# yxyxcyx/Real-Time-Recommendation-System-with-Feature-Store

Measured on AMD Instinct MI355X. Metric: user-item pairs scored/sec (train) + top-K queries/sec, emb_dim=128, higher is better.
Workload: dtype f32; 1 GPU; C2: MovieLens-1M two-tower train step, emb 128, batch 1024, 16 negatives, hidden [256,128], dropout 0.2, tau 0.05, Adam+clip; global_batch=1024, emb_dim=128, num_negatives=16, parallelism=dp1

## Files before the change

### include/rtrec_hip.h

```cpp
#ifndef RTREC_HIP_H
#define RTREC_HIP_H

#include <stddef.h>
#include <stdint.h>

#ifdef __cplusplus
extern "C" {
#endif

typedef enum {
    RT_OK = 0,
    RT_ERR_INVALID = -1,
    RT_ERR_UNSUPPORTED = -2,
    RT_ERR_WORKSPACE = -3,
    RT_ERR_HIP = -4
} rt_status;

typedef enum { RT_F32 = 0, RT_F16 = 1, RT_BF16 = 2 } rt_dtype;

typedef enum {
    RT_ACT_RELU = 0,
    RT_ACT_GELU = 1,
    RT_ACT_LEAKY_RELU = 2,
    RT_ACT_TANH = 3,
// ... 157 lines not shown
    const float* bn_gamma;
    float* dgamma;
    float* dbeta;
    const float* src; int64_t src_rows; int ld_src; const int64_t* ids;
    int prev_mode; int prev_act;
    const float* prev_mean; const float* prev_invstd;
    const float* prev_gamma; const float* prev_beta;
    float prev_drop_p; uint64_t prev_drop_seed; const uint64_t* seed_offset;
    float* g_prev;
    double* g_prev_stats;
    float* dsrc;
    int64_t seg_split;
    double* dbias_slots;
    const float* wt;
    int fuse_dz;
    const float* a_in;
    float* dw_part;
    const float* fold_src;
    float* fold_dst;
    int64_t fold_words;
    int fold_splits;
    int fold_in;
    const uint16_t* wt_planes;
} rt_linear_bwd_args;

int rt_linear_bwd_f32(const rt_linear_bwd_args* args, void* stream);
int rt_linear_bwd_dz_fused(const rt_linear_bwd_args* args, int n_args);
int rt_linear_bwd_dw_splits(const rt_linear_bwd_args* args, int n_args, int64_t* splits);
int rt_linear_bwd_dz_f32(const rt_linear_bwd_args* args, void* stream);
int rt_linear_bwd_dw_f32(const rt_linear_bwd_args* args, void* stream);
int rt_linear_fwd_f32_multi(const rt_linear_fwd_args* args, int n_args, void* stream);
int rt_linear_bwd_dz_f32_multi(const rt_linear_bwd_args* args, int n_args, void* stream);
int rt_linear_bwd_dw_f32_multi(const rt_linear_bwd_args* args, int n_args, void* stream);
int rt_linear_bwd_dw_f32_joint(const rt_linear_bwd_args* args, int n_args, void* stream);
int rt_linear_bwd_dw_joint_splits(const rt_linear_bwd_args* args, int n_args, int64_t* splits);

size_t rt_twotower_loss_workspace_bytes(int64_t b, int d);
int rt_twotower_loss_fwd_bwd(const void* u, const void* p, const void* q, int dtype, int64_t b,
                             int d, int n_neg, float inv_tau, const float* user_bias,
                             const float* item_bias, float w_explicit, float w_in_batch,
                             double* loss_out, float* du, float* dp, float* dq, float* d_user_bias,
                             float* d_item_bias, void* workspace, size_t workspace_bytes, void* stream);

int rt_twotower_loss_fwd(const void* u, const void* p, const void* q, int dtype, int64_t b, int d,
                         int n_neg, float inv_tau, const float* user_bias, const float* item_bias,
                         float w_explicit, float w_in_batch, double* loss_out, void* workspace,
                         size_t workspace_bytes, void* stream);

size_t rt_inbatch_loss_workspace_bytes(int64_t b, int64_t n_items, int d);
int rt_inbatch_loss_fwd_bwd(const void* u, const void* p, int dtype, int64_t b, int64_t n_items, int d,
                            int64_t label_offset, float inv_tau, double* loss_out, float* du, float* dp,
                            void* workspace, size_t workspace_bytes, void* stream);

int rt_similarity_f32(const float* u, const float* v, int64_t b, int d, float inv_tau,
                      const float* user_bias, const float* item_bias, float* out, void* stream);

#define RT_GRAD_FOLD_MAX 8
typedef struct {
    const float* part;
    int64_t dst_off;
    int64_t words;
    int splits;
    int tensor;
} rt_grad_fold;
int rt_grad_sqnorm(const float* grads, const int64_t* offsets, int n_tensors, double* sumsq_out,
// ... 54 lines not shown
```

### real-time-recommendation-system-with-feature-store_amd/csrc/loss.hip

```cpp
#include <float.h>

#include "rt_common.h"
#include "split3.h"

namespace rt {
size_t ib16_workspace_bytes(int64_t b, int64_t nx, int d);
int ib16_run(const void* u, const void* p, int dtype, int64_t b, int64_t nx, int d, int64_t off, float inv_tau,
             double* loss_out, float* du, float* dp, void* ws, size_t ws_bytes, hipStream_t st);
namespace loss {

typedef float f32x16 __attribute__((ext_vector_type(16)));
constexpr int RB = 32;
constexpr int kMaxD = 256;
constexpr int kMaxNeg = 64;
constexpr int NG = 16;


__device__ __forceinline__ int tile_row(int r, int h) { return (r & 3) + 8 * (r >> 2) + 4 * h; }

struct Args {
    const void* u; const void* p; const void* q;
    int64_t b; int d; int n_neg; float inv_tau;
    const float* ub; const float* ib;
    float we, wb;
    double* loss;
    float* du; float* dp; float* dq; float* dub; float* dib;
    float2* part;
    float* diag;
    float* expl;
    float* dposv;
    int64_t nx;
    int64_t off;
    int n_split;
    int ib_blocks;
    bool grad;
};

constexpr int SPAN = 256;
constexpr int LDP = 4;

template <typename T>
__device__ __forceinline__ float4 load4(const T* __restrict__ p) {
    if constexpr (sizeof(T) == 4) {
        return *reinterpret_cast<const float4*>(p);
    } else {
        const uint2 r = *reinterpret_cast<const uint2*>(p);
        const T* e = reinterpret_cast<const T*>(&r);
        return make_float4(to_f32(e[0]), to_f32(e[1]), to_f32(e[2]), to_f32(e[3]));
    }
}

template <int DP, typename T>
__device__ __forceinline__ void load_rows(const T* __restrict__ M, int64_t r0, int64_t n, int D,
                                          float4 (&v)[DP / 8]) {
    const int lane = threadIdx.x & 63;
#pragma unroll
    for (int u = 0; u < DP / 8; ++u) {
        const int e = lane + 64 * u;
// ... 171 lines not shown
            }
        }
    }
    wave_lds_sync();
    float se = expf(pos - mx);
    for (int j = 0; j < a.n_neg; ++j) se += expf(negs[w][j] - mx);
    const float lse = mx + logf(se);
    const float dpos = a.we * inv_b * (expf(pos - lse) - 1.f);
    if (lane == 0) {
        a.expl[i] = lse - pos;
        a.dposv[i] = dpos;
    }
    if (!a.grad) return;
    float duv[V];
#pragma unroll
    for (int t = 0; t < V; ++t) duv[t] = dpos * pv[t];
    for (int g0 = 0; g0 < a.n_neg; g0 += NG) {
        if (a.n_neg > NG) load_q(g0);
#pragma unroll
        for (int jj = 0; jj < NG; ++jj) {
            const int j = g0 + jj;
            if (j >= a.n_neg) break;
            const float dn = a.we * inv_b * expf(negs[w][j] - lse);
            float* dqr = a.dq + (i * a.n_neg + j) * D;
#pragma unroll
            for (int t = 0; t < V; ++t) {
                const int dd = lane + 64 * t;
                if (dd < D) {
                    duv[t] += dn * qv[jj][t];
                    dqr[dd] = dn * uv[t] * a.inv_tau;
                }
            }
        }
    }
#pragma unroll
    for (int t = 0; t < V; ++t) {
        const int dd = lane + 64 * t;
        if (dd < D) {
            a.du[i * D + dd] = duv[t] * a.inv_tau;
            a.dp[i * D + dd] = dpos * uv[t] * a.inv_tau;
        }
    }
}

__device__ __forceinline__ float combine_lse(const float2* part, int n_split, int64_t b, int64_t i) {
    float mm = -INFINITY;
    for (int s = 0; s < n_split; ++s) mm = fmaxf(mm, part[static_cast<int64_t>(s) * b + i].x);
    float ll = 0.f;
    for (int s = 0; s < n_split; ++s) {
        const float2 v = part[static_cast<int64_t>(s) * b + i];
        if (v.x != -INFINITY) ll += v.y * expf(v.x - mm);
    }
    return mm + logf(ll);
// ... 163 lines not shown
    hipLaunchKernelGGL((loss::loss_bwd_kernel<DP, T>), grid2, dim3(256), lds, st, a, wb_eff, true);
    return check_launch("loss_bwd_kernel");
}

template <typename T>
int launch_loss_d(const loss::Args& a, int dp32, dim3 grid1, dim3 grid2, float wb_eff, hipStream_t st) {
    switch (dp32) {
        case 32: return launch_loss<32, T>(a, grid1, grid2, wb_eff, st);
        case 64: return launch_loss<64, T>(a, grid1, grid2, wb_eff, st);
        case 96:
        case 128: return launch_loss<128, T>(a, grid1, grid2, wb_eff, st);
        default: return launch_loss<256, T>(a, grid1, grid2, wb_eff, st);
    }
}

size_t loss_ws_bytes(int64_t b, int64_t nx) {
    const int64_t n_split = (nx + loss::SPAN - 1) / loss::SPAN;
    return static_cast<size_t>(n_split) * b * sizeof(float2) + 3 * static_cast<size_t>(b) * sizeof(float);
}

int run_loss(const void* u, const void* p, const void* q, int dtype, int64_t b, int64_t nx, int64_t off, int d,
             int n_neg, float inv_tau, const float* ub, const float* ib, float we, float wb, double* loss_out,
             float* du, float* dp, float* dq, float* dub, float* dib, void* ws, size_t ws_bytes, void* stream,
             bool grad) {
    if (dtype != RT_F32 && dtype != RT_F16 && dtype != RT_BF16) return RT_ERR_INVALID;
    if (b <= 0 || d <= 0 || n_neg < 0 || !u || !p || !loss_out) return RT_ERR_INVALID;
    if (nx < b || off < 0 || off + b > nx) return RT_ERR_INVALID;
    if (d % 8 != 0 || d > loss::kMaxD || n_neg > loss::kMaxNeg) return RT_ERR_UNSUPPORTED;
    if (n_neg > 0 && !q) return RT_ERR_INVALID;
    if (grad && (!du || !dp || (n_neg > 0 && !dq))) return RT_ERR_INVALID;
    const int n_split = static_cast<int>((nx + loss::SPAN - 1) / loss::SPAN);
    if (!ws || ws_bytes < loss_ws_bytes(b, nx)) return RT_ERR_WORKSPACE;
    if ((reinterpret_cast<uintptr_t>(u) | reinterpret_cast<uintptr_t>(p)) & 15) return RT_ERR_INVALID;
    float2* part = reinterpret_cast<float2*>(ws);
    float* diag = reinterpret_cast<float*>(part + static_cast<size_t>(n_split) * b);
    const float wb_eff = n_neg > 0 ? wb : 1.f;
    const float we_eff = n_neg > 0 ? we : 0.f;
    const bool want_ib = wb_eff != 0.f;
    loss::Args a{u, p, q, b, d, n_neg, inv_tau, ub, ib, we_eff, wb_eff, loss_out, du, dp, dq, dub, dib, part, diag,
                 diag + b, diag + 2 * b, nx, off, n_split, want_ib ? n_split : 0, grad};
    hipStream_t st = as_stream(stream);
    if (grad && nx != b) {
        if (hipMemsetAsync(dp, 0, static_cast<size_t>(nx) * d * sizeof(float), st) != hipSuccess)
            return check_launch("hipMemsetAsync(dp)");
    }
    const int64_t big = nx > b ? nx : b;
    const int dp32 = (d + 31) / 32 * 32;
    const unsigned y2 = static_cast<unsigned>((big + loss::SPAN - 1) / loss::SPAN);
    const dim3 grid1(static_cast<unsigned>((b + loss::RB - 1) / loss::RB), a.ib_blocks + 8);
    const dim3 grid2(static_cast<unsigned>((big + loss::RB - 1) / loss::RB), want_ib ? y2 : 1,
                     (grad && want_ib) ? 2 : 1);
    switch (dtype) {
        case RT_F32: return launch_loss_d<float>(a, dp32, grid1, grid2, wb_eff, st);
        case RT_F16: return launch_loss_d<__half>(a, dp32, grid1, grid2, wb_eff, st);
        default: return launch_loss_d<__hip_bfloat16>(a, dp32, grid1, grid2, wb_eff, st);
    }
}
}

extern "C" size_t rt_twotower_loss_workspace_bytes(int64_t b, int d) {
    (void)d;
    if (b <= 0) return 256;
    return loss_ws_bytes(b, b) + 256;
// ... 11 lines not shown
    if (dtype == RT_F16 || dtype == RT_BF16) {
        if (b <= 0 || d <= 0 || !u || !p || !loss_out) return RT_ERR_INVALID;
        if (n_items < b || label_offset < 0 || label_offset + b > n_items) return RT_ERR_INVALID;
        if (d % 8 != 0 || d > loss::kMaxD) return RT_ERR_UNSUPPORTED;
        if ((du == nullptr) != (dp == nullptr)) return RT_ERR_INVALID;
        if ((reinterpret_cast<uintptr_t>(u) | reinterpret_cast<uintptr_t>(p)) & 15) return RT_ERR_INVALID;
        return ib16_run(u, p, dtype, b, n_items, d, label_offset, inv_tau, loss_out, du, dp, workspace,
                        workspace_bytes, as_stream(stream));
    }
    return run_loss(u, p, nullptr, dtype, b, n_items, label_offset, d, 0, inv_tau, nullptr, nullptr, 0.f, 1.f,
                    loss_out, du, dp, nullptr, nullptr, nullptr, workspace, workspace_bytes, stream, du != nullptr);
}


extern "C" int rt_twotower_loss_fwd_bwd(const void* u, const void* p, const void* q, int dtype, int64_t b, int d,
                                        int n_neg, float inv_tau, const float* user_bias, const float* item_bias,
                                        float w_explicit, float w_in_batch, double* loss_out, float* du, float* dp,
                                        float* dq, float* d_user_bias, float* d_item_bias, void* workspace,
                                        size_t workspace_bytes, void* stream) {
    return run_loss(u, p, q, dtype, b, b, 0, d, n_neg, inv_tau, user_bias, item_bias, w_explicit, w_in_batch,
                    loss_out, du, dp, dq, d_user_bias, d_item_bias, workspace, workspace_bytes, stream, true);
}

extern "C" int rt_twotower_loss_fwd(const void* u, const void* p, const void* q, int dtype, int64_t b, int d,
                                    int n_neg, float inv_tau, const float* user_bias, const float* item_bias,
                                    float w_explicit, float w_in_batch, double* loss_out, void* workspace,
                                    size_t workspace_bytes, void* stream) {
    return run_loss(u, p, q, dtype, b, b, 0, d, n_neg, inv_tau, user_bias, item_bias, w_explicit, w_in_batch,
                    loss_out, nullptr, nullptr, nullptr, nullptr, nullptr, workspace, workspace_bytes, stream, false);
}

extern "C" int rt_similarity_f32(const float* u, const float* v, int64_t b, int d, float inv_tau,
                                 const float* user_bias, const float* item_bias, float* out, void* stream) {
    if (b < 0 || d <= 0 || !u || !v || !out) return RT_ERR_INVALID;
    if ((user_bias == nullptr) != (item_bias == nullptr)) return RT_ERR_INVALID;
    if (b == 0) return RT_OK;
    hipLaunchKernelGGL(loss::similarity_kernel, dim3(static_cast<unsigned>((b + 3) / 4)), dim3(256), 0,
                       as_stream(stream), u, v, b, d, inv_tau, user_bias, item_bias, out);
    return check_launch("similarity_kernel");
}
```

### real-time-recommendation-system-with-feature-store_amd/csrc/mlp.hip

```cpp
#include "rt_common.h"
#include "split3.h"

namespace rt {
namespace mlp {

typedef float f32x16 __attribute__((ext_vector_type(16)));



constexpr float kNormEps = 1e-12f;

struct FwdLaunch {
    rt_linear_fwd_args a0, a1;
    unsigned split;
};
struct BwdLaunch {
    rt_linear_bwd_args a0, a1;
    unsigned split;
    int64_t rps0, rps1;
    unsigned tn0, tk0, tn1, tk1;
    bool vec0, vec1;
    int ngroups;
    unsigned ksplit = 1;
};
// ... 179 lines not shown
                s2 += v2[sl];
            }
            const double md = s1 / static_cast<double>(ms);
            double vd = s2 / static_cast<double>(ms) - md * md;
            vd = vd > 0.0 ? vd : 0.0;
            const float mean = static_cast<float>(md);
            const float invstd = static_cast<float>(1.0 / sqrt(vd + static_cast<double>(a.fin_eps)));
            const float var_f = static_cast<float>(ms > 1 ? vd * static_cast<double>(ms) / static_cast<double>(ms - 1) : vd);
            a.fin_save_mean[sg * n + c] = mean;
            if (a.fin_save_invstd) a.fin_save_invstd[sg * n + c] = invstd;
            if (a.fin_running_mean) {
                const float mo = a.fin_momentum;
                a.fin_running_mean[c] = (1.f - mo) * a.fin_running_mean[c] + mo * mean;
                a.fin_running_var[c] = (1.f - mo) * a.fin_running_var[c] + mo * var_f;
            }
        }
    }
    if (tid == 0 && a.fin_num_batches_tracked) *a.fin_num_batches_tracked += nseg;
}

constexpr int FM = 32;

__host__ __device__ __forceinline__ int pad8(int k) { return (k + 31) / 32 * 32; }

template <int TPW, bool KVEC, bool WPL>
__global__ __launch_bounds__(256) __attribute__((amdgpu_waves_per_eu(TPW == 1 ? 3 : 2))) void linear_fwd_kernel(FwdLaunch L) {
    static_assert(!WPL || (TPW == 1 && KVEC), "split-weight planes: one-tile waves, k % 4 == 0");
    const bool g1 = blockIdx.x >= L.split;
    const rt_linear_fwd_args& a = g1 ? L.a1 : L.a0;
    const unsigned bid = blockIdx.x - (g1 ? L.split : 0u);
    constexpr int NT = 4 * TPW;
    extern __shared__ __attribute__((aligned(16))) float sm[];
    const int k = a.k, n = a.n;
    const int kp = pad8(k), aplane = FM * kp, aw = 3 * aplane / 2;
    const int nch = kp / 8, am = ((nch & -nch) < 16 ? (nch & -nch) : 16) - 1;
    float* scale = sm;
    float* shift = scale + kp;
    float* As = shift + kp;
    uint16_t* const Ap = reinterpret_cast<uint16_t*>(As);
    float* rowpart = As + aw;
    int64_t* srow = reinterpret_cast<int64_t*>(rowpart + NT * FM);

    const int tid = threadIdx.x, lane = tid & 63, w = tid >> 6, h = lane >> 5, c32 = lane & 31;
    const int64_t row0 = static_cast<int64_t>(bid) * FM;
    const int64_t m = a.m;
    auto put_a = [&](int r, int c, float4 o) {
// ... 503 lines not shown
    uint4 pv[TPWK][3], pn[TPWK][3];
    const uint16_t* __restrict__ WtP = a.wt_planes;
    const int64_t tplane = static_cast<int64_t>(k) * n;
    auto load_p = [&](int s, uint4 (&dst)[TPWK][3]) {
#pragma unroll
        for (int i = 0; i < TPWK; ++i) {
            const int kk = (tb + w + 4 * i) * 32 + c32;
            const int nn = s + 8 * h;
            const bool ok = (tb + w + 4 * i) * 32 < k && kk < k && nn < n;
            const uint16_t* q = WtP + (ok ? static_cast<int64_t>(kk) * n + nn : 0);
#pragma unroll
            for (int p = 0; p < 3; ++p)
                dst[i][p] = ok ? *reinterpret_cast<const uint4*>(q + p * tplane) : make_uint4(0u, 0u, 0u, 0u);
        }
    };
    if constexpr (TPWK == 1) {
        if (a.g_prev || a.dsrc) {
            if constexpr (WPL) load_p(0, pn);
            else load_w(0, wn);
        }
    }

    const int l4 = n / 4;
    if (a.grad_mode == 0 && (n % 4) == 0 && l4 <= 64 && (l4 & (l4 - 1)) == 0 && np == n) {
        const int rpp = 64 / l4, sub = lane / l4, li = lane % l4, c = 4 * li;
        float4 lv[8], dv[8];
        float nr[8];
#pragma unroll
        for (int p = 0; p < 8; ++p) {
            const int r = w * 8 + p * rpp + sub;
            const int64_t gr = row0 + r;
            lv[p] = make_float4(0.f, 0.f, 0.f, 0.f);
            dv[p] = lv[p];
            nr[p] = 1.f;
            if (p * rpp < 8 && gr < m) {
                lv[p] = *reinterpret_cast<const float4*>(a.l2_out + gr * n + c);
                dv[p] = *reinterpret_cast<const float4*>(a.dout + gr * n + c);
                nr[p] = a.norms[gr];
            }
        }
#pragma unroll
        for (int p = 0; p < 8; ++p) {
            if (p * rpp >= 8) break;
            const int r = w * 8 + p * rpp + sub;
            const int64_t gr = row0 + r;
            float dot = lv[p].x * dv[p].x + lv[p].y * dv[p].y + lv[p].z * dv[p].z + lv[p].w * dv[p].w;
            for (int o = 1; o < l4; o <<= 1) dot += __shfl_xor(dot, o, 64);
            const bool big = nr[p] > kNormEps;
            const float inv = 1.f / (big ? nr[p] : kNormEps);
            float4 d = make_float4(0.f, 0.f, 0.f, 0.f);
            if (gr < m) {
                d.x = big ? (dv[p].x - lv[p].x * dot) * inv : dv[p].x * inv;
                d.y = big ? (dv[p].y - lv[p].y * dot) * inv : dv[p].y * inv;
                d.z = big ? (dv[p].z - lv[p].z * dot) * inv : dv[p].z * inv;
                d.w = big ? (dv[p].w - lv[p].w * dot) * inv : dv[p].w * inv;
                if (prim) st_act4(a.dz_ws + gr * n + c, d);
            }
            *reinterpret_cast<float4*>(Dz + r * ldz + c) = d;
        }
    } else if (a.grad_mode == 0) {
        for (int rr = w * 8; rr < w * 8 + 8; ++rr) {
            const int64_t gr = row0 + rr;
            if (gr < m) {
                float dot = 0.f;
                for (int c = lane; c < n; c += 64) dot += a.l2_out[gr * n + c] * a.dout[gr * n + c];
                dot = wave_sum(dot);
                const float nrm = a.norms[gr];
                const bool big = nrm > kNormEps;
// ... 795 lines not shown
}

static bool dz_fusable(const rt_linear_bwd_args& a) {
#ifdef RT_NO_DZ_FUSE
    return false;
#endif
    return a.fuse_dz && !a.g_prev && !a.dsrc && a.grad_mode >= 1 && a.grad_mode <= 3 &&
           act_is_piecewise_linear(a.act) && (a.n % 4) == 0 && a.g && a.z &&
           (reinterpret_cast<uintptr_t>(a.g) & 15) == 0 && (reinterpret_cast<uintptr_t>(a.z) & 15) == 0;
}
static bool all_dz_fusable(const rt_linear_bwd_args* args, int n_args) {
    for (int g = 0; g < n_args; ++g)
        if (!dz_fusable(args[g])) return false;
    return true;
}

static int validate_bwd(const rt_linear_bwd_args* args) {
    if (!args) return RT_ERR_INVALID;
    const rt_linear_bwd_args& a = *args;
    if (a.m < 0 || a.k <= 0 || a.n <= 0 || !a.w || !a.dw || !a.dz_ws || !a.src || a.ld_src < a.k)
        return RT_ERR_INVALID;
    const bool need_da = a.g_prev || a.dsrc;
    if (a.n > 2048 || (need_da && a.k > 512)) return RT_ERR_UNSUPPORTED;
    if (a.grad_mode == 0 && (!a.dout || !a.l2_out || !a.norms)) return RT_ERR_INVALID;
    if (a.grad_mode >= 1 && a.grad_mode <= 3 && (!a.g || !a.z)) return RT_ERR_INVALID;
    if ((a.grad_mode == 1 || a.grad_mode == 2) && (!a.g_stats || !a.save_mean || !a.save_invstd || !a.bn_gamma))
        return RT_ERR_INVALID;
    if (a.grad_mode < 0 || a.grad_mode > 3) return RT_ERR_INVALID;
    if (a.seg_split < 0 || (a.seg_split > 0 && (a.seg_split >= a.m || a.seg_split % mlp::FM != 0)))
        return RT_ERR_INVALID;
    if ((a.prev_mode == 1 || a.prev_mode == 2) &&
        (!a.prev_mean || !a.prev_invstd || !a.prev_gamma || !a.prev_beta))
        return RT_ERR_INVALID;
    if (a.fold_src && (!a.fold_dst || a.fold_words % 4 != 0 || a.fold_splits <= 0 || a.fold_in < 0 || a.fold_in > 1 ||
                       (reinterpret_cast<uintptr_t>(a.fold_src) & 15) || (reinterpret_cast<uintptr_t>(a.fold_dst) & 15)))
        return RT_ERR_INVALID;
    if (a.wt_planes && ((a.n % 8) != 0 || (reinterpret_cast<uintptr_t>(a.wt_planes) & 15))) return RT_ERR_INVALID;
    return RT_OK;
}

extern "C" int rt_linear_bwd_dz_f32_multi(const rt_linear_bwd_args* args, int n_args, void* stream) {
    if (!args || n_args < 1 || n_args > 2) return RT_ERR_INVALID;
    int tpwk = 1;
    size_t lds = 0;
    unsigned blocks[2] = {0u, 0u};
    bool wpl = true;
    for (int g = 0; g < n_args; ++g) {
// ... 388 lines not shown
```

### real-time-recommendation-system-with-feature-store_amd/rtrec_amd/models/fused.py

```python
from __future__ import annotations

import ctypes
import itertools
import os
from dataclasses import dataclass, field
from typing import List, Optional

import torch
import torch.nn as nn

from .. import native
from ..native import LinearBwdArgs, LinearFwdArgs, call, ptr
from ..profiling import TIMER

ACT_CODE = {nn.ReLU: 0, nn.GELU: 1, nn.LeakyReLU: 2, nn.Tanh: 3, nn.Sigmoid: 4}
ACT_NONE = 5

_seed_counter = itertools.count(1)


def act_code(mod: Optional[nn.Module]) -> int:
    if mod is None:
        return ACT_NONE
    for cls, code in ACT_CODE.items():
# ... 343 lines not shown
                ctx.norms = norms
            else:
                a.z_out = out.data_ptr()
            ctx.out = out
        layers.append(a)
    return ctx, layers


def chain_backward(blocks: List[Block], ctx: ChainCtx, dout: torch.Tensor, slab: ParamSlab,
                   want_dsrc: bool = False, seed_offset: Optional[torch.Tensor] = None,
                   stats_arena: Optional[torch.Tensor] = None, attach: bool = True) -> Optional[torch.Tensor]:
    layers, dsrc, keep = _backward_plan(blocks, ctx, dout, slab, want_dsrc, seed_offset, stats_arena, attach)
    st = _stream(dout)
    groups = [[a] for a in layers]
    if dw_joint_enabled():
        _launch_bwd_joint(groups, st, None)
        return dsrc
    keep += _plan_partials(groups, dout.device)
    for g in groups:
        _launch_bwd(g, st)
    return dsrc


def chain_backward_pair(first: tuple, second: tuple, fold_sink: Optional["FoldSink"] = None) -> None:
    l1, _, keep1 = _backward_plan(*first)
    l2, _, keep2 = _backward_plan(*second)
    st = _stream(first[2])
    if len(l1) == len(l2):
        groups = [[a, b] for a, b in zip(l1, l2)]
        if dw_joint_enabled():
            _launch_bwd_joint(groups, st, fold_sink)
            return
        keep1 += _plan_partials(groups, first[2].device)
    else:
        groups = [[a] for a in l1 + l2]
    for g in groups:
        _launch_bwd(g, st)


def dw_joint_enabled() -> bool:
    lib = native.lib()
    return (os.environ.get("RTREC_DW_LEGACY", "0") != "1" and hasattr(lib, "rt_linear_bwd_dw_f32_joint")
            and hasattr(lib, "rt_linear_bwd_dw_joint_splits") and hasattr(lib, "rt_linear_bwd_dz_fused"))


class FoldSink:

    def __init__(self, slab: ParamSlab):
        self.slab = slab
        self.buf: Optional[torch.Tensor] = None
        self.retired: list = []
        self.folds: list = []

    def begin(self) -> None:
        self.folds = []

# ... 80 lines not shown
    fused = hasattr(lib, "rt_linear_bwd_dz_fused") and lib.rt_linear_bwd_dz_fused(arr, len(group))
    if not fused:
        _launch_dz(group, st)
    _launch_dw(group, st)


def _launch_dz(group: list, st) -> None:
    da = [a.g_prev is not None or a.dsrc is not None for a in group]
    flops = sum((2.0 if d else 0.0) * a.m * a.k * a.n for a, d in zip(group, da))
    nbytes = sum(4.0 * (3 * a.m * a.n + (2 * a.m * a.k if d else 0) + a.n * a.k) for a, d in zip(group, da))
    with TIMER.region("linear_bwd_dz", flops=flops, bytes_=nbytes):
        call("rt_linear_bwd_dz_f32_multi", (LinearBwdArgs * len(group))(*group), len(group), st)


def _launch_dw(group: list, st) -> None:
    with TIMER.region("linear_bwd_dw", flops=sum(2.0 * a.m * a.k * a.n for a in group),
                      bytes_=sum(4.0 * (a.m * a.n + a.m * a.k + a.n * a.k) for a in group)):
        call("rt_linear_bwd_dw_f32_multi", (LinearBwdArgs * len(group))(*group), len(group), st)


def _backward_plan(blocks: List[Block], ctx: ChainCtx, dout: torch.Tensor, slab: ParamSlab,
                   want_dsrc: bool = False, seed_offset: Optional[torch.Tensor] = None,
                   stats_arena: Optional[torch.Tensor] = None, attach: bool = True):
    dev = dout.device
    dout = dout.contiguous()
    m = ctx.m
    L = len(blocks) - 1
    if attach:
        slab.attach_grads()
    dz_bufs = [torch.empty((m, b.linear.out_features), dtype=torch.float32, device=dev) for b in blocks]
    layers = []
    widths = [b.linear.out_features for b in blocks[:-1]]
    n_seg = 2 if ctx.seg_split else 1
    gst_arena = stats_arena if stats_arena is not None else \
        torch.zeros(stats_arena_size(blocks, n_seg), dtype=torch.float64, device=dev)
    gstats, off = [], 0
    for wdt in widths:
        gstats.append(gst_arena[off:off + n_seg * STAT_SLOTS * 2 * wdt])
        off += n_seg * STAT_SLOTS * 2 * wdt
    bslots = []
    for b in blocks:
        bslots.append(gst_arena[off:off + DBIAS_ROWS * b.linear.out_features])
        off += DBIAS_ROWS * b.linear.out_features
    gs: List[Optional[torch.Tensor]] = [None] * L
    dsrc = torch.empty((m, blocks[0].linear.in_features), dtype=torch.float32, device=dev) if want_dsrc else None
    keep = [dout, gst_arena] + dz_bufs
    for li in range(L, -1, -1):
        b = blocks[li]
        lin = b.linear
        a = LinearBwdArgs()
        a.m, a.k, a.n = m, lin.in_features, lin.out_features
        a.w = lin.weight.data_ptr()
        a.dw = slab.grad_of(lin.weight).data_ptr()
        a.dbias = slab.grad_of(lin.bias).data_ptr() if lin.bias is not None else None
        a.dbias_slots = bslots[li].data_ptr() if lin.bias is not None else None
        a.dz_ws = dz_bufs[li].data_ptr()
        a.seed_offset = seed_offset.data_ptr() if seed_offset is not None else None
        a.seg_split = ctx.seg_split
        if li == L:
            if ctx.normalize:
                a.grad_mode = 0
                a.dout = dout.data_ptr()
                a.l2_out = ctx.out.data_ptr()
                a.norms = ctx.norms.data_ptr()
            else:
                a.grad_mode = 3
                a.g = dout.data_ptr()
                a.z = dout.data_ptr()
                a.act = ACT_NONE
        else:
            a.grad_mode = ctx.bn_modes[li]
            a.g = gs[li].data_ptr()
            a.z = ctx.zs[li].data_ptr()
            a.act = b.act
            if b.bn is not None:
                a.g_stats = gstats[li].data_ptr()
                a.save_mean = ctx.save_mean[li].data_ptr()
                a.save_invstd = ctx.save_invstd[li].data_ptr()
                a.bn_gamma = b.bn.weight.data_ptr()
                a.dgamma = slab.grad_of(b.bn.weight).data_ptr()
                a.dbeta = slab.grad_of(b.bn.bias).data_ptr()
        if li == 0 and not want_dsrc:
            a.fuse_dz = 1
        if li == 0:
            a.src = ctx.src.data_ptr()
            a.src_rows = ctx.src.shape[0]
            a.ld_src = ctx.src.shape[1]
# ... 34 lines not shown
```

### real-time-recommendation-system-with-feature-store_amd/rtrec_amd/native.py

```python
from __future__ import annotations

import ctypes
import os
import threading
from typing import Optional

import torch

PKG_DIR = os.path.dirname(os.path.dirname(os.path.abspath(__file__)))
LIB_PATH = os.environ.get("RTREC_HIP_LIB", os.path.join(PKG_DIR, "lib", "librtrec_hip.so"))

RT_F32, RT_F16, RT_BF16 = 0, 1, 2
ACTS = {"relu": 0, "gelu": 1, "leaky_relu": 2, "tanh": 3, "sigmoid": 4, "none": 5}

c_i64 = ctypes.c_int64
c_int = ctypes.c_int
c_f32 = ctypes.c_float
c_u64 = ctypes.c_uint64
c_size = ctypes.c_size_t
vp = ctypes.c_void_p


class NativeUnavailable(RuntimeError):
    """librtrec_hip.so is missing or unusable (no CPU fallback exists)."""
# ... 16 lines not shown
        ("seed_offset", vp), ("z_out", vp), ("act", c_int), ("stats_out", vp), ("l2_out", vp), ("norms_out", vp),
        ("num_batches_tracked", vp), ("seg_split", c_i64), ("zero_buf", vp), ("zero_words", c_i64),
        ("wt_out", vp), ("a_out", vp),
        ("fin_save_mean", vp), ("fin_save_invstd", vp), ("fin_running_mean", vp), ("fin_running_var", vp),
        ("fin_num_batches_tracked", vp), ("fin_eps", c_f32), ("fin_momentum", c_f32), ("prev_final", c_int),
        ("w_planes", vp), ("wt_planes_out", vp), ("next_w", vp), ("next_w_planes", vp), ("next_n", c_int),
        ("next_k", c_int),
    ]


class LinearBwdArgs(ctypes.Structure):
    _fields_ = [
        ("m", c_i64), ("k", c_int), ("n", c_int), ("w", vp), ("dw", vp), ("dbias", vp), ("dz_ws", vp),
        ("grad_mode", c_int), ("dout", vp), ("l2_out", vp), ("norms", vp),
        ("g", vp), ("z", vp), ("act", c_int), ("g_stats", vp), ("save_mean", vp), ("save_invstd", vp),
        ("bn_gamma", vp), ("dgamma", vp), ("dbeta", vp),
        ("src", vp), ("src_rows", c_i64), ("ld_src", c_int), ("ids", vp),
        ("prev_mode", c_int), ("prev_act", c_int), ("prev_mean", vp), ("prev_invstd", vp),
        ("prev_gamma", vp), ("prev_beta", vp), ("prev_drop_p", c_f32), ("prev_drop_seed", c_u64),
        ("seed_offset", vp), ("g_prev", vp), ("g_prev_stats", vp), ("dsrc", vp), ("seg_split", c_i64),
        ("dbias_slots", vp), ("wt", vp), ("fuse_dz", c_int), ("a_in", vp), ("dw_part", vp),
        ("fold_src", vp), ("fold_dst", vp), ("fold_words", c_i64), ("fold_splits", c_int), ("fold_in", c_int),
        ("wt_planes", vp),
    ]


class GradFold(ctypes.Structure):
    _fields_ = [("part", vp), ("dst_off", c_i64), ("words", c_i64), ("splits", c_int), ("tensor", c_int)]


TOWER_MAX_LAYERS, TOWER_MAX_ROWS, TOWER_MAX_WIDTH = 8, 8, 512


class TowerLayer(ctypes.Structure):
    _fields_ = [("w", vp), ("bias", vp), ("k", c_int), ("n", c_int), ("act", c_int), ("bn_gamma", vp),
                ("bn_beta", vp), ("bn_mean", vp), ("bn_var", vp), ("bn_eps", c_f32)]


class TowerInferArgs(ctypes.Structure):
    _fields_ = [("src", vp), ("src_rows", c_i64), ("ld_src", c_int), ("ids", vp), ("m", c_int),
                ("n_layers", c_int), ("layers", TowerLayer * TOWER_MAX_LAYERS), ("normalize", c_int),
                ("out", vp), ("norms_out", vp)]


ONLINE_MAX_EXCL_SOURCES = 2

# ... 33 lines not shown
                                            vp]),
    "rt_topk_sample_rank": (c_int, [c_int, c_i64, c_i64, vp]),
    "rt_topk_sample_threshold": (c_int, [vp, c_int, c_i64, c_int, vp, vp]),
    "rt_flatip_topk_shard_search": (c_int, [vp, c_i64, vp, c_i64, c_int, c_int, c_int, vp, c_i64, vp, vp, vp,
                                            c_size, vp]),
    "rt_sample_negatives": (c_int, [vp, vp, c_i64, vp, c_i64, c_i64, c_int, c_u64, vp, vp, vp]),
    "rt_feeder_batch": (c_int, [vp, vp, vp, vp, c_i64, vp, vp, vp]),
    "rt_feeder_commit": (c_int, [vp, vp, c_i64, vp, vp]),
    "rt_linear_fwd_f32": (c_int, [ctypes.POINTER(LinearFwdArgs), vp]),
    "rt_linear_bwd_f32": (c_int, [ctypes.POINTER(LinearBwdArgs), vp]),
    "rt_linear_bwd_dz_f32": (c_int, [ctypes.POINTER(LinearBwdArgs), vp]),
    "rt_linear_bwd_dz_fused": (c_int, [ctypes.POINTER(LinearBwdArgs), c_int]),
    "rt_linear_bwd_dw_splits": (c_int, [ctypes.POINTER(LinearBwdArgs), c_int, ctypes.POINTER(c_i64)]),
    "rt_linear_bwd_dw_f32": (c_int, [ctypes.POINTER(LinearBwdArgs), vp]),
    "rt_linear_fwd_f32_multi": (c_int, [ctypes.POINTER(LinearFwdArgs), c_int, vp]),
    "rt_linear_bwd_dz_f32_multi": (c_int, [ctypes.POINTER(LinearBwdArgs), c_int, vp]),
    "rt_linear_bwd_dw_f32_multi": (c_int, [ctypes.POINTER(LinearBwdArgs), c_int, vp]),
    "rt_linear_bwd_dw_f32_joint": (c_int, [ctypes.POINTER(LinearBwdArgs), c_int, vp]),
    "rt_linear_bwd_dw_joint_splits": (c_int, [ctypes.POINTER(LinearBwdArgs), c_int, ctypes.POINTER(c_i64)]),
    "rt_tower_infer_f32": (c_int, [ctypes.POINTER(TowerInferArgs), vp]),
    "rt_twotower_loss_workspace_bytes": (c_size, [c_i64, c_int]),
    "rt_twotower_loss_fwd_bwd": (c_int, [vp, vp, vp, c_int, c_i64, c_int, c_int, c_f32, vp, vp, c_f32,
                                         c_f32, vp, vp, vp, vp, vp, vp, vp, c_size, vp]),
    "rt_twotower_loss_fwd": (c_int, [vp, vp, vp, c_int, c_i64, c_int, c_int, c_f32, vp, vp, c_f32, c_f32,
                                     vp, vp, c_size, vp]),
    "rt_inbatch_loss_workspace_bytes": (c_size, [c_i64, c_i64, c_int]),
    "rt_inbatch_loss_fwd_bwd": (c_int, [vp, vp, c_int, c_i64, c_i64, c_int, c_i64, c_f32, vp, vp, vp, vp, c_size, vp]),
    "rt_similarity_f32": (c_int, [vp, vp, c_i64, c_int, c_f32, vp, vp, vp, vp]),
    "rt_grad_sqnorm": (c_int, [vp, vp, c_int, vp, vp, vp, vp]),
    "rt_grad_sqnorm_fold": (c_int, [vp, vp, c_int, vp, vp, vp, ctypes.POINTER(GradFold), c_int, vp]),
    "rt_clip_adam_step": (c_int, [vp, vp, vp, vp, c_i64, vp, c_int, c_f32, c_f32, vp, c_f32, c_f32, c_f32,
                                  c_f32, c_int, vp, vp, c_i64, vp]),
    "rt_l2_augment_f32": (c_int, [vp, c_i64, c_int, vp, c_int, c_int, vp]),
    "rt_l2_finish_f32": (c_int, [vp, c_int, vp, c_int, c_int, c_i64, c_int, vp, vp, c_int, vp, vp, vp, c_i64, vp]),
    "rt_exclusion_bitmap": (c_int, [vp, vp, c_i64, vp, c_i64, c_i64, vp, c_i64, vp]),
    "rt_rank_metrics": (c_int, [vp, c_i64, c_int, vp, vp, vp, c_i64, vp, vp, vp, c_i64, vp, c_int, c_i64, vp, vp,
                                vp, vp]),
    "rt_rank_metrics_reduce": (c_int, [vp, vp, c_i64, c_int, vp, c_i64, vp, vp]),
}

RT_METRICS_MAX_K = 16

_lib = None
_lock = threading.Lock()
_load_error: Optional[str] = None
MISSING: list = []
# ... 72 lines not shown
```

### real-time-recommendation-system-with-feature-store_amd/rtrec_amd/training/fused_step.py

```python
from __future__ import annotations

import ctypes
import itertools
from typing import Dict, Optional

import torch

from .. import kernels, native
from ..models.fused import (FoldSink, blocks_from_sequential, chain_backward, chain_backward_pair, chain_forward,
                            chain_forward_pair, stats_arena_size)
from ..models.two_tower import TwoTowerModel
from ..native import call, ptr
from ..profiling import TIMER


_STEP_SEEDS = itertools.count(0x5EED)


def _adjacent_or_cat(a: torch.Tensor, b: torch.Tensor) -> torch.Tensor:
    if (a.is_contiguous() and b.is_contiguous() and a.dtype == b.dtype and a.device == b.device
            and a.untyped_storage().data_ptr() == b.untyped_storage().data_ptr()
            and b.data_ptr() == a.data_ptr() + a.numel() * a.element_size()):
        return torch.as_strided(a, (a.numel() + b.numel(),), (1,))
    return torch.cat([a.reshape(-1), b.reshape(-1)])


class FusedTrainStep:
    def __init__(self, model: TwoTowerModel, lr: float = 1e-3, weight_decay: float = 1e-5, max_norm: float = 1.0,
                 betas=(0.9, 0.999), eps: float = 1e-8, explicit_weight: float = 0.7,
                 in_batch_weight: float = 0.3, process_group=None, dropout_seed: Optional[int] = None):
        self.model = model
        self.pg = process_group
        self.slab = model.slab()
# ... 102 lines not shown
            if pos_ids is not None:
                item_src, item_ids = pos_src, _adjacent_or_cat(pos_ids, neg_ids)
            else:
                item_src, item_ids = torch.cat([pos_src, neg_src]), None
            pq, u = chain_forward_pair((ib, item_src, item_ids, True, so, self.a_pqf, b, self._sb_pos),
                                       (ub, user_src, user_ids, True, so, self.a_uf, 0, self._sb_user),
                                       zero_buf=self.small)
            p_out, q_out = pq.out[:b], pq.out[b:]
        else:
            p = chain_forward(ib, pos_src, pos_ids, seed_offset=so, stats_arena=self.a_pf, zero_buf=self.small,
                              seed_base=self._sb_pos)
            q = chain_forward(ib, neg_src, neg_ids, seed_offset=so, stats_arena=self.a_nf,
                              seed_base=self._sb_neg) if (neg_src is not None) else None
            p_out, q_out = p.out, (q.out if q is not None else None)
        if not merged:
            s_u.wait_stream(main)
            with torch.cuda.stream(s_u):
                u = chain_forward(ub, user_src, user_ids, seed_offset=so, stats_arena=self.a_uf,
                                  seed_base=self._sb_user)
            main.wait_stream(s_u)
        d = u.out.shape[1]
        n_neg = (q_out.shape[0] // b) if q_out is not None else 0
        du = torch.empty_like(u.out)
        if merged:
            dpq = torch.empty_like(pq.out)
            dp, dq = dpq[:b], dpq[b:]
        else:
            dp = torch.empty_like(p_out)
            dq = torch.empty_like(q_out) if q_out is not None else None
        ws = self._loss_workspace(native.lib().rt_twotower_loss_workspace_bytes(b, d))
        ubias, ibias = m.user_bias, m.item_bias
        with TIMER.region("loss_fwd_bwd", flops=6.0 * b * b * d + 6.0 * b * (n_neg + 1) * d,
                          bytes_=4.0 * d * (4 * b + 2 * b * n_neg)):
            call("rt_twotower_loss_fwd_bwd", ptr(u.out), ptr(p_out), ptr(q_out) if q_out is not None else None, 0,
                 b, d, n_neg, 1.0 / m.temperature, ptr(ubias), ptr(ibias), self.we, self.wb, ptr(self.loss_buf),
                 ptr(du), ptr(dp), ptr(dq),
                 ptr(slab.grad_of(ubias)) if ubias is not None else None,
                 ptr(slab.grad_of(ibias)) if ibias is not None else None, ptr(ws), ws.numel(), st)
        self._fold.begin()
        if merged:
            chain_backward_pair((ib, pq, dpq, slab, False, so, self.a_pqb, False),
                                (ub, u, du, slab, False, so, self.a_ub, False),
                                fold_sink=self._fold if self.pg is None else None)
        else:
            s_u.wait_stream(main)
            with torch.cuda.stream(s_u):
                chain_backward(ub, u, du, slab, seed_offset=so, stats_arena=self.a_ub, attach=False)
            s_p.wait_stream(main)
            with torch.cuda.stream(s_p):
                chain_backward(ib, p, dp, slab, seed_offset=so, stats_arena=self.a_pb, attach=False)
            if q is not None:
                chain_backward(ib, q, dq, slab, seed_offset=so, stats_arena=self.a_nb, attach=False)
            main.wait_stream(s_p)
        main.wait_stream(s_u)

    def _loss_workspace(self, nbytes: int) -> torch.Tensor:
        if self._loss_ws is None or self._loss_ws.numel() < nbytes:
            if self._loss_ws is not None:
                self._loss_ws_retired.append(self._loss_ws)
# ... 185 lines not shown
```

Before: 4.917 billion pairs/s.

## Pass negative-item output gradients as rank-1 coefficients instead of dense slab

The loss kernel now writes one scalar coefficient per (user, negative) pair rather than a full dq row of dim d. The item-tower backward dz kernel rebuilds each negative's output gradient on the fly as coef * u[row / n_neg] * inv_tau. This removes the write and re-read of the b*n_neg*d dq tensor. It adds a shuffle and a gather from the user embeddings inside the backward kernel, and the path can be turned off through an environment variable.

After: 4.937 billion pairs/s (median of 6 runs). No clear change (+0.4%).

```diff
diff --git a/include/rtrec_hip.h b/include/rtrec_hip.h
--- a/include/rtrec_hip.h
+++ b/include/rtrec_hip.h
@@ -203,6 +203,11 @@
     int fold_splits;
     int fold_in;
     const uint16_t* wt_planes;
+    const float* dout_coef;
+    const float* dout_vec;
+    int64_t dout_r1_from;
+    int dout_group;
+    float dout_scale;
 } rt_linear_bwd_args;
 
 int rt_linear_bwd_f32(const rt_linear_bwd_args* args, void* stream);
@@ -222,6 +227,12 @@
                              const float* item_bias, float w_explicit, float w_in_batch,
                              double* loss_out, float* du, float* dp, float* dq, float* d_user_bias,
                              float* d_item_bias, void* workspace, size_t workspace_bytes, void* stream);
+int rt_twotower_loss_fwd_bwd_coef(const void* u, const void* p, const void* q, int dtype, int64_t b,
+                                  int d, int n_neg, float inv_tau, const float* user_bias,
+                                  const float* item_bias, float w_explicit, float w_in_batch,
+                                  double* loss_out, float* du, float* dp, float* dq_coef,
+                                  float* d_user_bias, float* d_item_bias, void* workspace,
+                                  size_t workspace_bytes, void* stream);
 
 int rt_twotower_loss_fwd(const void* u, const void* p, const void* q, int dtype, int64_t b, int d,
                          int n_neg, float inv_tau, const float* user_bias, const float* item_bias,
diff --git a/real-time-recommendation-system-with-feature-store_amd/csrc/loss.hip b/real-time-recommendation-system-with-feature-store_amd/csrc/loss.hip
--- a/real-time-recommendation-system-with-feature-store_amd/csrc/loss.hip
+++ b/real-time-recommendation-system-with-feature-store_amd/csrc/loss.hip
@@ -34,6 +34,7 @@
     int n_split;
     int ib_blocks;
     bool grad;
+    float* dq_coef;
 };
 
 constexpr int SPAN = 256;
@@ -251,13 +252,14 @@
             const int j = g0 + jj;
             if (j >= a.n_neg) break;
             const float dn = a.we * inv_b * expf(negs[w][j] - lse);
-            float* dqr = a.dq + (i * a.n_neg + j) * D;
+            float* dqr = a.dq_coef ? nullptr : a.dq + (i * a.n_neg + j) * D;
+            if (a.dq_coef && lane == 0) a.dq_coef[i * a.n_neg + j] = dn;
 #pragma unroll
             for (int t = 0; t < V; ++t) {
                 const int dd = lane + 64 * t;
                 if (dd < D) {
                     duv[t] += dn * qv[jj][t];
-                    dqr[dd] = dn * uv[t] * a.inv_tau;
+                    if (dqr) dqr[dd] = dn * uv[t] * a.inv_tau;
                 }
             }
         }
@@ -467,13 +469,14 @@
 int run_loss(const void* u, const void* p, const void* q, int dtype, int64_t b, int64_t nx, int64_t off, int d,
              int n_neg, float inv_tau, const float* ub, const float* ib, float we, float wb, double* loss_out,
              float* du, float* dp, float* dq, float* dub, float* dib, void* ws, size_t ws_bytes, void* stream,
-             bool grad) {
+             bool grad, float* dq_coef = nullptr) {
     if (dtype != RT_F32 && dtype != RT_F16 && dtype != RT_BF16) return RT_ERR_INVALID;
     if (b <= 0 || d <= 0 || n_neg < 0 || !u || !p || !loss_out) return RT_ERR_INVALID;
     if (nx < b || off < 0 || off + b > nx) return RT_ERR_INVALID;
     if (d % 8 != 0 || d > loss::kMaxD || n_neg > loss::kMaxNeg) return RT_ERR_UNSUPPORTED;
     if (n_neg > 0 && !q) return RT_ERR_INVALID;
-    if (grad && (!du || !dp || (n_neg > 0 && !dq))) return RT_ERR_INVALID;
+    if (grad && (!du || !dp || (n_neg > 0 && !dq && !dq_coef))) return RT_ERR_INVALID;
+    if (dq && dq_coef) return RT_ERR_INVALID;
     const int n_split = static_cast<int>((nx + loss::SPAN - 1) / loss::SPAN);
     if (!ws || ws_bytes < loss_ws_bytes(b, nx)) return RT_ERR_WORKSPACE;
     if ((reinterpret_cast<uintptr_t>(u) | reinterpret_cast<uintptr_t>(p)) & 15) return RT_ERR_INVALID;
@@ -483,7 +486,7 @@
     const float we_eff = n_neg > 0 ? we : 0.f;
     const bool want_ib = wb_eff != 0.f;
     loss::Args a{u, p, q, b, d, n_neg, inv_tau, ub, ib, we_eff, wb_eff, loss_out, du, dp, dq, dub, dib, part, diag,
-                 diag + b, diag + 2 * b, nx, off, n_split, want_ib ? n_split : 0, grad};
+                 diag + b, diag + 2 * b, nx, off, n_split, want_ib ? n_split : 0, grad, dq_coef};
     hipStream_t st = as_stream(stream);
     if (grad && nx != b) {
         if (hipMemsetAsync(dp, 0, static_cast<size_t>(nx) * d * sizeof(float), st) != hipSuccess)
@@ -541,6 +544,17 @@
                     loss_out, du, dp, dq, d_user_bias, d_item_bias, workspace, workspace_bytes, stream, true);
 }
 
+extern "C" int rt_twotower_loss_fwd_bwd_coef(const void* u, const void* p, const void* q, int dtype, int64_t b, int d,
+                                             int n_neg, float inv_tau, const float* user_bias,
+                                             const float* item_bias, float w_explicit, float w_in_batch,
+                                             double* loss_out, float* du, float* dp, float* dq_coef,
+                                             float* d_user_bias, float* d_item_bias, void* workspace,
+                                             size_t workspace_bytes, void* stream) {
+    return run_loss(u, p, q, dtype, b, b, 0, d, n_neg, inv_tau, user_bias, item_bias, w_explicit, w_in_batch,
+                    loss_out, du, dp, nullptr, d_user_bias, d_item_bias, workspace, workspace_bytes, stream, true,
+                    dq_coef);
+}
+
 extern "C" int rt_twotower_loss_fwd(const void* u, const void* p, const void* q, int dtype, int64_t b, int d,
                                     int n_neg, float inv_tau, const float* user_bias, const float* item_bias,
                                     float w_explicit, float w_in_batch, double* loss_out, void* workspace,
diff --git a/real-time-recommendation-system-with-feature-store_amd/csrc/mlp.hip b/real-time-recommendation-system-with-feature-store_amd/csrc/mlp.hip
--- a/real-time-recommendation-system-with-feature-store_amd/csrc/mlp.hip
+++ b/real-time-recommendation-system-with-feature-store_amd/csrc/mlp.hip
@@ -225,6 +225,10 @@
 constexpr int FM = 32;
 
 __host__ __device__ __forceinline__ int pad8(int k) { return (k + 31) / 32 * 32; }
+__host__ __device__ __forceinline__ bool dz_mode0_fast(int n) {
+    const int l4 = n / 4;
+    return (n % 4) == 0 && l4 >= 1 && l4 <= 64 && (l4 & (l4 - 1)) == 0 && pad8(n) == n;
+}
 
 template <int TPW, bool KVEC, bool WPL>
 __global__ __launch_bounds__(256) __attribute__((amdgpu_waves_per_eu(TPW == 1 ? 3 : 2))) void linear_fwd_kernel(FwdLaunch L) {
@@ -774,10 +778,18 @@
     }
 
     const int l4 = n / 4;
-    if (a.grad_mode == 0 && (n % 4) == 0 && l4 <= 64 && (l4 & (l4 - 1)) == 0 && np == n) {
+    if (a.grad_mode == 0 && dz_mode0_fast(n)) {
         const int rpp = 64 / l4, sub = lane / l4, li = lane % l4, c = 4 * li;
         float4 lv[8], dv[8];
         float nr[8];
+        const float* __restrict__ coef = a.dout_coef;
+        const int64_t r1_from = coef ? a.dout_r1_from : m;
+        const uint32_t r1_group = static_cast<uint32_t>(a.dout_group);
+        float cfl = 0.f;
+        {
+            const int64_t gr = row0 + w * 8 + (lane & 7);
+            if (gr >= r1_from && gr < m) cfl = coef[gr - r1_from];
+        }
 #pragma unroll
         for (int p = 0; p < 8; ++p) {
             const int r = w * 8 + p * rpp + sub;
@@ -787,7 +799,12 @@
             nr[p] = 1.f;
             if (p * rpp < 8 && gr < m) {
                 lv[p] = *reinterpret_cast<const float4*>(a.l2_out + gr * n + c);
-                dv[p] = *reinterpret_cast<const float4*>(a.dout + gr * n + c);
+                if (gr >= r1_from) {
+                    const uint32_t t = static_cast<uint32_t>(gr - r1_from);
+                    dv[p] = *reinterpret_cast<const float4*>(a.dout_vec + static_cast<int64_t>(t / r1_group) * n + c);
+                } else {
+                    dv[p] = *reinterpret_cast<const float4*>(a.dout + gr * n + c);
+                }
                 nr[p] = a.norms[gr];
             }
         }
@@ -796,6 +813,15 @@
             if (p * rpp >= 8) break;
             const int r = w * 8 + p * rpp + sub;
             const int64_t gr = row0 + r;
+            if (coef) {
+                const float cf = __shfl(cfl, p * rpp + sub, 64);
+                if (gr >= r1_from) {
+                    dv[p].x = (cf * dv[p].x) * a.dout_scale;
+                    dv[p].y = (cf * dv[p].y) * a.dout_scale;
+                    dv[p].z = (cf * dv[p].z) * a.dout_scale;
+                    dv[p].w = (cf * dv[p].w) * a.dout_scale;
+                }
+            }
             float dot = lv[p].x * dv[p].x + lv[p].y * dv[p].y + lv[p].z * dv[p].z + lv[p].w * dv[p].w;
             for (int o = 1; o < l4; o <<= 1) dot += __shfl_xor(dot, o, 64);
             const bool big = nr[p] > kNormEps;
@@ -1637,7 +1663,15 @@
         return RT_ERR_INVALID;
     const bool need_da = a.g_prev || a.dsrc;
     if (a.n > 2048 || (need_da && a.k > 512)) return RT_ERR_UNSUPPORTED;
-    if (a.grad_mode == 0 && (!a.dout || !a.l2_out || !a.norms)) return RT_ERR_INVALID;
+    if (a.dout_coef) {
+        if (a.grad_mode != 0 || !mlp::dz_mode0_fast(a.n)) return RT_ERR_UNSUPPORTED;
+        if (!a.dout_vec || (reinterpret_cast<uintptr_t>(a.dout_vec) & 15) || a.dout_group < 1 ||
+            a.dout_r1_from < 0 || a.dout_r1_from > a.m)
+            return RT_ERR_INVALID;
+        if (a.m - a.dout_r1_from > INT32_MAX) return RT_ERR_UNSUPPORTED;
+    }
+    const bool dense_dout = !a.dout_coef || a.dout_r1_from > 0;
+    if (a.grad_mode == 0 && ((dense_dout && !a.dout) || !a.l2_out || !a.norms)) return RT_ERR_INVALID;
     if (a.grad_mode >= 1 && a.grad_mode <= 3 && (!a.g || !a.z)) return RT_ERR_INVALID;
     if ((a.grad_mode == 1 || a.grad_mode == 2) && (!a.g_stats || !a.save_mean || !a.save_invstd || !a.bn_gamma))
         return RT_ERR_INVALID;
diff --git a/real-time-recommendation-system-with-feature-store_amd/rtrec_amd/models/fused.py b/real-time-recommendation-system-with-feature-store_amd/rtrec_amd/models/fused.py
--- a/real-time-recommendation-system-with-feature-store_amd/rtrec_amd/models/fused.py
+++ b/real-time-recommendation-system-with-feature-store_amd/rtrec_amd/models/fused.py
@@ -389,16 +389,30 @@
     return dsrc
 
 
+@dataclass
+class Rank1Dout:
+    dense: torch.Tensor
+    coef: torch.Tensor
+    vec: torch.Tensor
+    group: int
+    scale: float
+
+
+def dq_coef_enabled(d: int) -> bool:
+    return os.environ.get("RTREC_DQ_SLAB", "0") != "1" and d in (32, 64, 128, 256)
+
+
 def chain_backward_pair(first: tuple, second: tuple, fold_sink: Optional["FoldSink"] = None) -> None:
     l1, _, keep1 = _backward_plan(*first)
     l2, _, keep2 = _backward_plan(*second)
-    st = _stream(first[2])
+    d0 = first[2].dense if isinstance(first[2], Rank1Dout) else first[2]
+    st = _stream(d0)
     if len(l1) == len(l2):
         groups = [[a, b] for a, b in zip(l1, l2)]
         if dw_joint_enabled():
             _launch_bwd_joint(groups, st, fold_sink)
             return
-        keep1 += _plan_partials(groups, first[2].device)
+        keep1 += _plan_partials(groups, d0.device)
     else:
         groups = [[a] for a in l1 + l2]
     for g in groups:
@@ -525,6 +539,11 @@
 def _backward_plan(blocks: List[Block], ctx: ChainCtx, dout: torch.Tensor, slab: ParamSlab,
                    want_dsrc: bool = False, seed_offset: Optional[torch.Tensor] = None,
                    stats_arena: Optional[torch.Tensor] = None, attach: bool = True):
+    r1 = dout if isinstance(dout, Rank1Dout) else None
+    if r1 is not None:
+        if not ctx.normalize:
+            raise NotImplementedError("a rank-1 output gradient needs the normalised last layer")
+        dout = r1.dense
     dev = dout.device
     dout = dout.contiguous()
     m = ctx.m
@@ -548,6 +567,8 @@
     gs: List[Optional[torch.Tensor]] = [None] * L
     dsrc = torch.empty((m, blocks[0].linear.in_features), dtype=torch.float32, device=dev) if want_dsrc else None
     keep = [dout, gst_arena] + dz_bufs
+    if r1 is not None:
+        keep += [r1.coef, r1.vec]
     for li in range(L, -1, -1):
         b = blocks[li]
         lin = b.linear
@@ -566,6 +587,9 @@
                 a.dout = dout.data_ptr()
                 a.l2_out = ctx.out.data_ptr()
                 a.norms = ctx.norms.data_ptr()
+                if r1 is not None:
+                    a.dout_coef, a.dout_vec = r1.coef.data_ptr(), r1.vec.data_ptr()
+                    a.dout_r1_from, a.dout_group, a.dout_scale = dout.shape[0], r1.group, r1.scale
             else:
                 a.grad_mode = 3
                 a.g = dout.data_ptr()
diff --git a/real-time-recommendation-system-with-feature-store_amd/rtrec_amd/native.py b/real-time-recommendation-system-with-feature-store_amd/rtrec_amd/native.py
--- a/real-time-recommendation-system-with-feature-store_amd/rtrec_amd/native.py
+++ b/real-time-recommendation-system-with-feature-store_amd/rtrec_amd/native.py
@@ -62,6 +62,7 @@
         ("dbias_slots", vp), ("wt", vp), ("fuse_dz", c_int), ("a_in", vp), ("dw_part", vp),
         ("fold_src", vp), ("fold_dst", vp), ("fold_words", c_i64), ("fold_splits", c_int), ("fold_in", c_int),
         ("wt_planes", vp),
+        ("dout_coef", vp), ("dout_vec", vp), ("dout_r1_from", c_i64), ("dout_group", c_int), ("dout_scale", c_f32),
     ]
 
 
@@ -141,6 +142,8 @@
     "rt_twotower_loss_workspace_bytes": (c_size, [c_i64, c_int]),
     "rt_twotower_loss_fwd_bwd": (c_int, [vp, vp, vp, c_int, c_i64, c_int, c_int, c_f32, vp, vp, c_f32,
                                          c_f32, vp, vp, vp, vp, vp, vp, vp, c_size, vp]),
+    "rt_twotower_loss_fwd_bwd_coef": (c_int, [vp, vp, vp, c_int, c_i64, c_int, c_int, c_f32, vp, vp, c_f32,
+                                              c_f32, vp, vp, vp, vp, vp, vp, vp, c_size, vp]),
     "rt_twotower_loss_fwd": (c_int, [vp, vp, vp, c_int, c_i64, c_int, c_int, c_f32, vp, vp, c_f32, c_f32,
                                      vp, vp, c_size, vp]),
     "rt_inbatch_loss_workspace_bytes": (c_size, [c_i64, c_i64, c_int]),
diff --git a/real-time-recommendation-system-with-feature-store_amd/rtrec_amd/training/fused_step.py b/real-time-recommendation-system-with-feature-store_amd/rtrec_amd/training/fused_step.py
--- a/real-time-recommendation-system-with-feature-store_amd/rtrec_amd/training/fused_step.py
+++ b/real-time-recommendation-system-with-feature-store_amd/rtrec_amd/training/fused_step.py
@@ -7,8 +7,8 @@
 import torch
 
 from .. import kernels, native
-from ..models.fused import (FoldSink, blocks_from_sequential, chain_backward, chain_backward_pair, chain_forward,
-                            chain_forward_pair, stats_arena_size)
+from ..models.fused import (FoldSink, Rank1Dout, blocks_from_sequential, chain_backward, chain_backward_pair,
+                            chain_forward, chain_forward_pair, dq_coef_enabled, stats_arena_size)
 from ..models.two_tower import TwoTowerModel
 from ..native import call, ptr
 from ..profiling import TIMER
@@ -157,7 +157,13 @@
         d = u.out.shape[1]
         n_neg = (q_out.shape[0] // b) if q_out is not None else 0
         du = torch.empty_like(u.out)
-        if merged:
+        coef = merged and n_neg > 0 and pq.normalize and dq_coef_enabled(d)
+        dq_coef = None
+        if coef:
+            dp, dq = torch.empty_like(p_out), None
+            dq_coef = torch.empty(b * n_neg, dtype=torch.float32, device=self.dev)
+            dpq = Rank1Dout(dp, dq_coef, u.out, n_neg, 1.0 / m.temperature)
+        elif merged:
             dpq = torch.empty_like(pq.out)
             dp, dq = dpq[:b], dpq[b:]
         else:
@@ -167,9 +173,10 @@
         ubias, ibias = m.user_bias, m.item_bias
         with TIMER.region("loss_fwd_bwd", flops=6.0 * b * b * d + 6.0 * b * (n_neg + 1) * d,
                           bytes_=4.0 * d * (4 * b + 2 * b * n_neg)):
-            call("rt_twotower_loss_fwd_bwd", ptr(u.out), ptr(p_out), ptr(q_out) if q_out is not None else None, 0,
+            call("rt_twotower_loss_fwd_bwd_coef" if coef else "rt_twotower_loss_fwd_bwd", ptr(u.out), ptr(p_out),
+                 ptr(q_out) if q_out is not None else None, 0,
                  b, d, n_neg, 1.0 / m.temperature, ptr(ubias), ptr(ibias), self.we, self.wb, ptr(self.loss_buf),
-                 ptr(du), ptr(dp), ptr(dq),
+                 ptr(du), ptr(dp), ptr(dq_coef) if coef else ptr(dq),
                  ptr(slab.grad_of(ubias)) if ubias is not None else None,
                  ptr(slab.grad_of(ibias)) if ibias is not None else None, ptr(ws), ws.numel(), st)
         self._fold.begin()
```
